# dcherednik/atracdenc

Hardware: AMD Instinct MI355X
Metric: ATRAC3 1024-sample stereo frames/sec (higher is better)
Workload: dtype f32; 1 GPU; ATRAC3 LP2 132 kbps stereo, 64 streams x 64 frames = 4096 frames per GPU per step (BASELINE configs[1]), 'noise' PCM resident in HBM, frames written to HBM (PCIe excluded); streams_per_gpu=64, frame_bytes=384, input=noise, tonal_components=True, parallelism=streams/1, launch=1 process x 1 GPU(s), one host thread and one at3hip context per device, collectives=none (no RCCL); start/stop barrier only

## Files before the change

### atracdenc_amd/csrc/at3_k_gain.hpp

```cpp
#pragma once
#include "at3_common.hpp"

namespace at3 {

struct GainParams {
    const float* sub;
    GainRec* rec;
    cpx* bins;
    BandState* state;
    Curve* curves;
    int n_blocks;
    int f0;
    int js;
    int n_streams;
    int literal;
};

constexpr int kLowCutBin = 38;

__device__ inline void median3_32(const float* in, float* out)
{
    for (int i = 0; i < 32; ++i) {
        const int lo = i > 0 ? i - 1 : 0;
        const int hi = i < 31 ? i + 1 : 31;
        if (hi - lo == 1) {
            out[i] = fmaxf(in[lo], in[hi]);
        } else {
            const float a = in[lo], b = in[lo + 1], c = in[hi];
            out[i] = fmaxf(fminf(a, b), fminf(fmaxf(a, b), c));
        }
    }
}

__device__ inline float curve_target(const float* in, const float* filtered)
{
    float maxRaw = 0.0f;
    for (int i = 0; i < 32; ++i) maxRaw = fmaxf(maxRaw, in[i]);
    float bestLevel = 0.0f;
    int bestEnd = -1;
    for (int j = 0; j + 3 <= 32; ++j) {
        const float minVal = fminf(fminf(filtered[j], filtered[j + 1]), filtered[j + 2]);
        if (minVal > bestLevel) {
            bestLevel = minVal;
            bestEnd = j + 2;
        }
    }
    float plateau = 0.0f;
    bool release = false;
    if (!(bestLevel < 1e-6f)) {
        plateau = bestLevel;
        while (bestEnd + 1 < 32 && filtered[bestEnd + 1] >= bestLevel) ++bestEnd;
        if (bestEnd < 31) {
            if (in[31] < bestLevel * 0.1f) {
                release = true;
            } else {
                bool anyHigh = false;
                for (int i = bestEnd + 1; i < 32; ++i)
                    if (in[i] >= bestLevel * 0.7f) {
                        anyHigh = true;
                        break;
                    }
                release = !anyHigh && (in[31] < bestLevel * 0.5f);
            }
        }
    }
    const bool usePlateau = plateau > 1e-6f && !release && plateau >= maxRaw * 0.4f;
    return usePlateau ? plateau : in[31];
}

__device__ __forceinline__ int irfft_pad(int i) { return i + (i >> 5); }

template <bool Z1>
__device__ __forceinline__ void bfly4_inv_sparse(f2& x0, f2& x1, f2& x2, f2& x3, f2 w1, f2 w3)
{
    const f2 s2 = pk_cmul(x3, w3);
    const f2 f0 = x0;
    if (Z1) {
        x2 = f0 - s2;
        x0 = f0 + s2;
        x1 = pk_sub_ib(f0, s2);
        x3 = pk_add_ib(f0, s2);
    } else {
        const f2 s0 = pk_cmul(x1, w1);
        const f2 s3 = s0 + s2, s4 = s0 - s2;
        x2 = f0 - s3;
        x0 = f0 + s3;
        x1 = pk_add_ib(f0, s4);
        x3 = pk_sub_ib(f0, s4);
    }
}

template <int KAPPA>
__device__ __forceinline__ void irfft_pass_2_8(cpx* F, const cpx* tw, int lane)
{
    cpx* B = F + 33 * lane + KAPPA;
    f2 x[16];
    const int r0 = (lane >> 4) + 4 * ((lane >> 2) & 3) + 16 * (lane & 3);
#pragma unroll
    for (int i = 0; i < 16; ++i) {
        const int r = r0 + 64 * (i >> 2);
        const bool nz = (i & 3) == 0 ? r >= 38 : (i & 3) == 1 ? r == 0 : (i & 3) == 3 ? r <= 218 : false;
        x[i] = f2{0.0f, 0.0f};
        if ((i & 3) != 2 && nz) x[i] = ld2(B + 2 * i);
    }
    const f2 a1 = ld2(tw + 256 * KAPPA), a3 = ld2(tw + 768 * KAPPA);
    bfly4_inv_sparse<false>(x[0], x[1], x[2], x[3], a1, a3);
#pragma unroll
    for (int g = 1; g < 4; ++g) bfly4_inv_sparse<true>(x[4 * g], x[4 * g + 1], x[4 * g + 2], x[4 * g + 3], a1, a3);
#pragma unroll
    for (int j = 0; j < 4; ++j) {
        const int k = KAPPA + 2 * j;
        bfly4<true>(x[j], x[j + 4], x[j + 8], x[j + 12], ld2(tw + 64 * k), ld2(tw + 128 * k), ld2(tw + 192 * k));
    }
#pragma unroll
    for (int i = 0; i < 16; ++i) st2(B + 2 * i, x[i]);
}

struct Tw32_128 {
    f2 a[3];
    f2 w[4][3];
};
__device__ __forceinline__ Tw32_128 irfft_tw_32_128(const cpx (*g)[128], int v)
{
    Tw32_128 t;
    t.a[0] = ld2(&g[0][v]);
    t.a[1] = ld2(&g[1][v]);
    t.a[2] = ld2(&g[2][v]);
#pragma unroll
    for (int j = 0; j < 4; ++j) {
        t.w[j][0] = ld2(&g[3 + 3 * j][v]);
        t.w[j][1] = ld2(&g[4 + 3 * j][v]);
        t.w[j][2] = ld2(&g[5 + 3 * j][v]);
    }
    return t;
}
__device__ __forceinline__ void irfft_pass_32_128(cpx* F, const Tw32_128& t, int v)
{
    const int k = v & 31, G2 = v >> 5;
    cpx* B = F + 528 * G2 + k;
    f2 x[16];
#pragma unroll
    for (int i = 0; i < 16; ++i) x[i] = ld2(B + 33 * i);
#pragma unroll
    for (int g = 0; g < 4; ++g) bfly4<true>(x[4 * g], x[4 * g + 1], x[4 * g + 2], x[4 * g + 3], t.a[0], t.a[1], t.a[2]);
#pragma unroll
    for (int j = 0; j < 4; ++j) bfly4<true>(x[j], x[j + 4], x[j + 8], x[j + 12], t.w[j][0], t.w[j][1], t.w[j][2]);
#pragma unroll
    for (int i = 0; i < 16; ++i) st2(B + 33 * i, x[i]);
}

template <int NT>
struct Tw512 {
    f2 w[512 / NT][3];
};
template <int NT>
__device__ __forceinline__ Tw512<NT> irfft_tw_512(const cpx (*g)[128], int tid)
{
    static_assert(NT == 128, "Tables::gain_tw is laid out for 128 work-items");
    Tw512<NT> t;
#pragma unroll
    for (int u = 0; u < 512 / NT; ++u) {
        t.w[u][0] = ld2(&g[15 + 3 * u][tid]);
        t.w[u][1] = ld2(&g[16 + 3 * u][tid]);
        t.w[u][2] = ld2(&g[17 + 3 * u][tid]);
    }
    return t;
}
template <int NT>
__device__ __forceinline__ void irfft_pass_512(cpx* F, const Tw512<NT>& t, int tid)
{
#pragma unroll
    for (int u0 = 0; u0 < 512 / NT; u0 += 4) {
        f2 x[4][4];
        cpx* B[4];
#pragma unroll
        for (int u = 0; u < 4; ++u) {
            B[u] = F + irfft_pad(tid + NT * (u0 + u));
#pragma unroll
            for (int q = 0; q < 4; ++q) x[u][q] = ld2(B[u] + 528 * q);
        }
#pragma unroll
        for (int u = 0; u < 4; ++u) bfly4<true>(x[u][0], x[u][1], x[u][2], x[u][3], t.w[u0 + u][0], t.w[u0 + u][1], t.w[u0 + u][2]);
#pragma unroll
        for (int u = 0; u < 4; ++u) {
            st2(B[u] + 528, x[u][1]);
            st2(B[u] + 1056, x[u][2]);
        }
    }
}

template <int CTRL>
__device__ __forceinline__ double dpp_f64_zero_fill(double v)
{
    const uint64_t b = (uint64_t)__double_as_longlong(v);
    const uint32_t lo = (uint32_t)AT3_DPP((uint32_t)b, CTRL, true), hi = (uint32_t)AT3_DPP((uint32_t)(b >> 32), CTRL, true);
    return __longlong_as_double((long long)(((uint64_t)hi << 32) | lo));
}
__device__ __forceinline__ double row_scan_add_f64(double v)
{
    v += dpp_f64_zero_fill<0x111>(v);
    v += dpp_f64_zero_fill<0x112>(v);
    v += dpp_f64_zero_fill<0x114>(v);
    v += dpp_f64_zero_fill<0x118>(v);
    return v;
}
constexpr int kGainBins = 220;

constexpr int kSpecRowStride = 18;
constexpr int kSpecItemBytes = 2432;
struct SpecItemLds {
    union {
        cpx x[16 * kSpecRowStride];
        double e[304];
    };
};
static_assert(sizeof(SpecItemLds) == kSpecItemBytes, "SpecItemLds layout");

__global__ __launch_bounds__(64) void k_gain_spec(GainParams p, const Tables* T, int n_items)
{
    __shared__ __attribute__((aligned(16))) SpecItemLds s_item[4];
    const int lane = threadIdx.x, row = lane >> 4, L = lane & 15;
    SpecItemLds& S = s_item[row];
    const int nfr = p.n_blocks - p.f0;
    const int quads = (nfr + 3) >> 2;
    int wg = blockIdx.x;
    const int band = wg % 3; wg /= 3;
    const int ch = wg % 2; wg /= 2;
    const int fr = 4 * (wg % quads) + row;
    const int s = wg / quads;
    const bool valid = fr < nfr;
    const int f = p.f0 + (valid ? fr : nfr - 1);
    const int item = (((s * nfr) + (f - p.f0)) * 2 + ch) * 3 + band;
    (void)n_items;
    const int cb = f - 1;
    const size_t sublen = (size_t)(p.n_blocks + 2) * 256;
    const float* sb0 = p.sub + ((size_t)s * 8 + 0 * 4 + band) * sublen + (size_t)(cb + 2) * 256 - 128;
    const float* sb1 = p.sub + ((size_t)s * 8 + 1 * 4 + band) * sublen + (size_t)(cb + 2) * 256 - 128;
    GainRec* rec = p.rec + (((size_t)s * p.n_blocks + f) * 2 + ch) * 3 + band;
    cpx* bins = p.bins + (size_t)item * kGainBins;

    f2 a[16];
    {
        f2 raw[16], rb[16], win[16];
#pragma unroll
        for (int t = 0; t < 16; ++t) {
            const int i = L + 16 * t;
            raw[t] = *reinterpret_cast<const f2*>((p.js || ch == 0 ? sb0 : sb1) + 2 * i);
            if (p.js) rb[t] = *reinterpret_cast<const f2*>(sb1 + 2 * i);
        }
#pragma unroll
        for (int t = 0; t < 16; ++t) win[t] = ld2(&T->spec16_win[t][L]);
        __builtin_amdgcn_sched_barrier(0);
#pragma unroll
        for (int t = 0; t < 16; ++t) {
            f2 v = raw[t];
            if (p.js) v = (ch == 0) ? (v + rb[t]) * mk2(0.5f, 0.5f) : (v - rb[t]) * mk2(0.5f, 0.5f);
            a[4 * (t & 3) + (t >> 2)] = v * win[t];
        }
    }
    f2 tw_l[15];
#pragma unroll
    for (int q = 0; q < 15; ++q) tw_l[q] = ld2(&T->spec16_tw[q][L]);
    __builtin_amdgcn_sched_barrier(0);
    {
        const f2 w0 = ld2(&T->tw256[0]);
#pragma unroll
        for (int q3 = 0; q3 < 4; ++q3) bfly4<false>(a[4 * q3], a[4 * q3 + 1], a[4 * q3 + 2], a[4 * q3 + 3], w0, w0, w0);
#pragma unroll
        for (int k = 0; k < 4; ++k)
            bfly4<false>(a[k], a[k + 4], a[k + 8], a[k + 12], ld2(&T->tw256[16 * k]), ld2(&T->tw256[32 * k]), ld2(&T->tw256[48 * k]));
    }
    f2 b[16];
    {
#pragma unroll
        for (int r = 0; r < 16; ++r) st2(&S.x[r * kSpecRowStride + L], a[r]);
        wave_sync();
        const float4* src = reinterpret_cast<const float4*>(&S.x[L * kSpecRowStride]);
#pragma unroll
        for (int m = 0; m < 8; ++m) {
            const float4 v = src[m];
            b[2 * m] = mk2(v.x, v.y);
            b[2 * m + 1] = mk2(v.z, v.w);
        }
        wave_sync();
    }
    {
        const f2 u1 = tw_l[0], u2 = tw_l[1], u3 = tw_l[2];
#pragma unroll
        for (int q1 = 0; q1 < 4; ++q1) bfly4<false>(b[q1], b[q1 + 4], b[q1 + 8], b[q1 + 12], u1, u2, u3);
#pragma unroll
        for (int j = 0; j < 4; ++j) bfly4<false>(b[4 * j], b[4 * j + 1], b[4 * j + 2], b[4 * j + 3], tw_l[3 + 3 * j], tw_l[4 + 3 * j], tw_l[5 + 3 * j]);
    }
    f2 fa[8], fb[8];
    f2 f128 = mk2(0.0f, 0.0f);
    {
        const int partner = 4 * ((lane & 48) | ((16 - L) & 15));
#pragma unroll
        for (int jj = 0; jj < 8; ++jj) {
            const int je = 15 - jj;
            const f2 pe = b[(je >> 2) + 4 * (je & 3)];
            f2 other;
            other.x = __uint_as_float((uint32_t)__builtin_amdgcn_ds_bpermute(partner, (int)__float_as_uint(pe.x)));
            other.y = __uint_as_float((uint32_t)__builtin_amdgcn_ds_bpermute(partner, (int)__float_as_uint(pe.y)));
            if (jj > 0) {
                const int j0 = 16 - jj;
                const f2 own = b[(j0 >> 2) + 4 * (j0 & 3)];
                if (L == 0) other = own;
            }
            const f2 fpk = b[(jj >> 2) + 4 * (jj & 3)];
            const cpx stw = T->spec16_stw[jj][L];
            const float fnr = other.x, fni = -other.y;
            const float f1r = fpk.x + fnr, f1i = fpk.y + fni;
            const float f2r = fpk.x - fnr, f2i = fpk.y - fni;
            const float twr = f2r * stw.r - f2i * stw.i, twi = f2r * stw.i + f2i * stw.r;
            fa[jj] = mk2((f1r + twr) * 0.5f, (f1i + twi) * 0.5f);
            fb[jj] = mk2((f1r - twr) * 0.5f, (twi - f1i) * 0.5f);
        }
        if (L == 0) {
            const f2 f0 = b[0];
            fa[0] = mk2(f0.x + f0.y, 0.0f);
            fb[0] = mk2(f0.x - f0.y, 0.0f);
        }
        {
            const f2 fpk = b[2];
            const cpx stw = T->spec16_stw[8][L];
            const float fnr = fpk.x, fni = -fpk.y;
            const float f1r = fpk.x + fnr, f1i = fpk.y + fni;
            const float f2r = fpk.x - fnr, f2i = fpk.y - fni;
            const float twr = f2r * stw.r - f2i * stw.i, twi = f2r * stw.i + f2i * stw.r;
            f128 = mk2((f1r - twr) * 0.5f, (twi - f1i) * 0.5f);
        }
    }
    if (valid) {
#pragma unroll
        for (int jj = 0; jj < 8; ++jj) {
            const int k = L + 16 * jj;
            if (k >= kLowCutBin) st2(&bins[k - kLowCutBin], fa[jj]);
            st2(&bins[256 - k - kLowCutBin], fb[jj]);
        }
        if (L == 0) st2(&bins[128 - kLowCutBin], f128);
    }
    bool fast_done = false;
    {
        const double h1 = (double)T->hpf_w[1], h2 = (double)T->hpf_w[2];
        double et = 0.0, ef = 0.0;
#pragma unroll
        for (int jj = 0; jj < 8; ++jj) {
            const int k = L + 16 * jj;
            const double ea = (double)fa[jj].x * fa[jj].x + (double)fa[jj].y * fa[jj].y;
            const double eb = (double)fb[jj].x * fb[jj].x + (double)fb[jj].y * fb[jj].y;
            et += ea;
            et += eb;
            const double wa = (k < kLowCutBin) ? 0.0 : (k == kLowCutBin) ? ea * h1 * h1 : (k == kLowCutBin + 1) ? ea * h2 * h2 : ea;
            ef += wa;
            ef += eb;
        }
        if (L == 0) {
            const double e128 = (double)f128.x * f128.x + (double)f128.y * f128.y;
            et += e128;
            ef += e128;
        }
        et = row_scan_add_f64(et);
        ef = row_scan_add_f64(ef);
        bool need = false;
        float hfr = 0.0f;
        if (L == 15) {
            if (et > 0.0 && ef > 0.0) {
                const double r = ef / et;
                hfr = (float)r;
                if (!(hfr >= 1e-30f)) {
                    need = true;
                } else {
                    const uint32_t hb = __float_as_uint(hfr);
                    const double below = ((double)__uint_as_float(hb - 1u) + (double)hfr) * 0.5, above = ((double)hfr + (double)__uint_as_float(hb + 1u)) * 0.5;
                    const double margin = r * 4e-13;
                    need = !(r - below > margin && above - r > margin);
                }
            }
        }
        if (p.literal || __ballot(need && valid) != 0ull) {
            fast_done = false;
        } else {
            if (valid && L == 15) rec->hfr = hfr;
            fast_done = true;
        }
    }
    if (fast_done) return;
    {
#pragma unroll
        for (int jj = 0; jj < 8; ++jj) {
            const int k = L + 16 * jj;
            S.e[k] = (double)fa[jj].x * fa[jj].x + (double)fa[jj].y * fa[jj].y;
            S.e[256 - k] = (double)fb[jj].x * fb[jj].x + (double)fb[jj].y * fb[jj].y;
        }
        if (L == 0) S.e[128] = (double)f128.x * f128.x + (double)f128.y * f128.y;
        for (int k = 257 + L; k < 304; k += 16) S.e[k] = 0.0;
    }
    wave_sync();
    double acc = 0.0;
    if (lane < 8) {
        const int it = lane >> 1, kind = lane & 1;
        const double* E = s_item[it].e;
        const double h1 = (double)T->hpf_w[1], h2 = (double)T->hpf_w[2];
        if (kind == 1) {
            acc += E[kLowCutBin] * h1 * h1;
            acc += E[kLowCutBin + 1] * h2 * h2;
        }
        const double* src = E + (kind ? kLowCutBin + 2 : 0);
        for (int k0 = 0; k0 < 256; k0 += 16) {
            double v[16];
#pragma unroll
            for (int i = 0; i < 16; ++i) v[i] = src[k0 + i];
#pragma unroll
            for (int i = 0; i < 16; ++i) acc += v[i];
        }
        acc += src[256];
    }
    const uint64_t ab = (uint64_t)__double_as_longlong(acc);
    const int alo = (int)(uint32_t)ab, ahi = (int)(uint32_t)(ab >> 32);
    const uint64_t fb64 = (uint64_t)(uint32_t)__builtin_amdgcn_ds_bpermute(4 * (2 * row + 1), alo) |
                          ((uint64_t)(uint32_t)__builtin_amdgcn_ds_bpermute(4 * (2 * row + 1), ahi) << 32);
    const uint64_t tb64 = (uint64_t)(uint32_t)__builtin_amdgcn_ds_bpermute(4 * (2 * row), alo) |
                          ((uint64_t)(uint32_t)__builtin_amdgcn_ds_bpermute(4 * (2 * row), ahi) << 32);
    if (valid && L == 0) {
        const double totalE = __longlong_as_double((long long)tb64), filtE = __longlong_as_double((long long)fb64);
        rec->hfr = (totalE > 0.0) ? (float)(filtE / totalE) : 0.0f;
    }
}

struct GainLds {
    cpx f[2048 + 64];
};

__global__ __launch_bounds__(128) void k_gain_analysis(GainParams p, const Tables* __restrict__ T)
{
    __shared__ __attribute__((aligned(16))) GainLds s_item[1];
    const int tid = threadIdx.x, wave = __builtin_amdgcn_readfirstlane((int)(threadIdx.x >> 6)), lane = threadIdx.x & 63;
    GainLds& L = s_item[0];
    const int nfr = p.n_blocks - p.f0;
    const bool valid = true;
    int wg = blockIdx.x;
    const size_t item = blockIdx.x;
    const int band = wg % 3; wg /= 3;
    const int ch = wg % 2; wg /= 2;
    const int f = p.f0 + wg % nfr;
    const int s = wg / nfr;
    GainRec* rec = p.rec + (((size_t)s * p.n_blocks + f) * 2 + ch) * 3 + band;
    const float hfr = rec->hfr;
    const cpx* bins = p.bins + item * kGainBins;
    const int k0 = kLowCutBin + tid, k1 = kLowCutBin + 128 + tid;
    const cpx bin0 = bins[tid];
    const cpx bin1 = bins[k1 <= 256 ? 128 + tid : tid];
    const cpx stw_in0 = T->stw2048[k0 - 1];
    const cpx stw_in1 = T->stw2048[k1 - 1 < 1024 ? k1 - 1 : 1023];
    const float hpf1 = T->hpf_w[1], hpf2 = T->hpf_w[2];
    __builtin_amdgcn_sched_barrier(0);
    if (hfr < 0.05f) return;
    __builtin_amdgcn_sched_barrier(0);
    const Tw32_128 tw_b = irfft_tw_32_128(T->gain_tw, tid);
    const Tw512<128> tw_c = irfft_tw_512<128>(T->gain_tw, tid);
    __builtin_amdgcn_sched_barrier(0);
#pragma unroll
    for (int q = 0; q < 2; ++q) {
        const int k = q ? k1 : k0;
        const cpx fr = q ? bin1 : bin0;
        cpx fk;
        const float scale = 8.0f;
        if (k == 256) {
            fk.r = fr.r * scale * 0.5f;
            fk.i = 0.0f;
        } else if (k >= kLowCutBin + 2) {
            fk.r = fr.r * scale;
            fk.i = fr.i * scale;
        } else {
            const float w = (k == kLowCutBin) ? hpf1 : hpf2;
            fk.r = fr.r * scale * w;
            fk.i = fr.i * scale * w;
        }
        const cpx fok = cmul(fk, q ? stw_in1 : stw_in0);
        cpx a, b, nb;
        a.r = fk.r + fok.r; a.i = fk.i + fok.i;
        b.r = fk.r - fok.r; b.i = -(fk.i - fok.i);
        nb.r = 0.0f - b.r; nb.i = 0.0f - b.i;
        if (k <= 256) {
            const int pa = fft_leaf_pos<2048>(k);
            L.f[irfft_pad(pa)] = a;
            L.f[irfft_pad(pa) + 1] = a;
            const int pb = fft_leaf_pos<2048>(2048 - k);
            L.f[irfft_pad(pb) - 1] = b;
            L.f[irfft_pad(pb)] = nb;
        }
    }
    __syncthreads();

    if (wave == 0) irfft_pass_2_8<0>(L.f, T->tw2048, lane);
    else irfft_pass_2_8<1>(L.f, T->tw2048, lane);
    __syncthreads();

    irfft_pass_32_128(L.f, tw_b, tid);
    __syncthreads();

    irfft_pass_512<128>(L.f, tw_c, tid);
    __syncthreads();


    const float norm = 1.0f / 4096.0f;
    float* s_micro = reinterpret_cast<float*>(L.f);
#pragma unroll
    for (int q = 0; q < 2; ++q) {
        const int n = tid + 128 * q;
        const int c = (n & 3) | ((n & 0xc) << 1) | ((n & 0x10) >> 2) | (n & 0xe0);
        cpx* src = L.f + 528 + 4 * c + (c >> 3);
        float acc = 0.0f;
#pragma unroll
        for (int i = 0; i < 4; ++i) {
            const f2 v = ld2(src + i) * norm;
            const f2 sq = v * v;
            st2(src + i, sq);
            acc += sq.x;
            acc += sq.y;
        }
        acc /= 8;
        s_micro[c] = sqrtf(acc);
    }
    __syncthreads();
    if (tid < 32) {
        const cpx* src = L.f + 528 + 33 * lane;
        f2 x[32];
#pragma unroll
        for (int i = 0; i < 32; ++i) x[i] = ld2(src + i);
        float acc = 0.0f;
#pragma unroll
        for (int i = 0; i < 32; ++i) {
            acc += x[i].x;
            acc += x[i].y;
        }
        acc /= 64;
        rec->gain[lane] = sqrtf(acc);
    } else if (wave == 1 && lane < 32) {
        const float4 ma = *reinterpret_cast<const float4*>(s_micro + 8 * lane), mb = *reinterpret_cast<const float4*>(s_micro + 8 * lane + 4);
        float m[8] = {ma.x, ma.y, ma.z, ma.w, mb.x, mb.y, mb.z, mb.w};
#pragma unroll
        for (int i = 1; i < 8; ++i) {
#pragma unroll
            for (int k = i; k > 0; --k) {
                const float lo = fminf(m[k - 1], m[k]), hi = fmaxf(m[k - 1], m[k]);
                m[k - 1] = lo;
                m[k] = hi;
            }
        }
        rec->lo[lane] = m[2];
        rec->hi[lane] = m[6];
    }
}

constexpr int kGa1RowStride = 18;
constexpr int kGa1RowSlots = 16 * kGa1RowStride + 16;
constexpr int kGa1SubStride = 33;
struct Gain1Lds {
    union {
        cpx x[4 * kGa1RowSlots];
        struct {
            cpx out[32 * kGa1SubStride];
            float micro[256];
        };
    };
};
static_assert(sizeof(Gain1Lds) <= 10240, "sixteen items per CU");

struct PermPair {
    int a, b;
};
__device__ __forceinline__ PermPair perm32_swap(int a, int b)
{
    const auto r = __builtin_amdgcn_permlane32_swap(a, b, false, false);
    return PermPair{(int)r[0], (int)r[1]};
}
__device__ __forceinline__ PermPair perm16_swap(int a, int b)
{
    const auto r = __builtin_amdgcn_permlane16_swap(a, b, false, false);
    return PermPair{(int)r[0], (int)r[1]};
}
template <bool WIDE>
__device__ __forceinline__ void swap_f2(f2& a, f2& b)
{
    const PermPair x = WIDE ? perm32_swap((int)__float_as_uint(a.x), (int)__float_as_uint(b.x)) : perm16_swap((int)__float_as_uint(a.x), (int)__float_as_uint(b.x));
    const PermPair y = WIDE ? perm32_swap((int)__float_as_uint(a.y), (int)__float_as_uint(b.y)) : perm16_swap((int)__float_as_uint(a.y), (int)__float_as_uint(b.y));
    a = mk2(__uint_as_float((uint32_t)x.a), __uint_as_float((uint32_t)y.a));
    b = mk2(__uint_as_float((uint32_t)x.b), __uint_as_float((uint32_t)y.b));
}

__global__ __launch_bounds__(64) AT3_WAVES_PER_EU(4) void k_gain_analysis1(GainParams p, const Tables* T)
{
    __shared__ __attribute__((aligned(16))) Gain1Lds L;
    const int lane = threadIdx.x, R = lane >> 4, j = lane & 15;
    const int nfr = p.n_blocks - p.f0;
    int wg = blockIdx.x;
    const size_t item = blockIdx.x;
    const int band = wg % 3; wg /= 3;
    const int ch = wg % 2; wg /= 2;
    const int f = p.f0 + wg % nfr;
    const int s = wg / nfr;
    GainRec* rec = p.rec + (((size_t)s * p.n_blocks + f) * 2 + ch) * 3 + band;
    const float hfr = rec->hfr;
    if (hfr < 0.05f) return;
    const cpx* bins = p.bins + item * kGainBins;
    const cpx* tw = T->tw2048;

#define AT3_STAGE() __builtin_amdgcn_sched_barrier(0)
    const int r0 = (lane >> 4) + 4 * ((lane >> 2) & 3) + 16 * (lane & 3);
    cpx ba[4], bb[4], sa[4], sb[4], b256 = {0.0f, 0.0f}, s256 = {0.0f, 0.0f};
#pragma unroll
    for (int q = 0; q < 4; ++q) {
        const int ka = r0 + 64 * q, kb = 256 - r0 - 64 * q;
        const int kac = ka >= kLowCutBin ? ka : kLowCutBin, kbc = kb >= kLowCutBin ? kb : kLowCutBin;
        ba[q] = bins[kac - kLowCutBin];
        sa[q] = T->stw2048[kac - 1];
        bb[q] = bins[kbc - kLowCutBin];
        sb[q] = T->stw2048[kbc - 1];
    }
    if (lane == 0) {
        b256 = bins[256 - kLowCutBin];
        s256 = T->stw2048[255];
    }
    const float hpf1 = T->hpf_w[1], hpf2 = T->hpf_w[2];
    f2 a1[2], a3[2], w8[2][4][3];
#pragma unroll
    for (int kappa = 0; kappa < 2; ++kappa) {
        a1[kappa] = ld2(tw + 256 * kappa);
        a3[kappa] = ld2(tw + 768 * kappa);
#pragma unroll
        for (int jj = 0; jj < 4; ++jj) {
            const int k = kappa + 2 * jj;
            w8[kappa][jj][0] = ld2(tw + 64 * k);
            w8[kappa][jj][1] = ld2(tw + 128 * k);
            w8[kappa][jj][2] = ld2(tw + 192 * k);
        }
    }
    f2 twb[15];
#pragma unroll
    for (int sl = 0; sl < 15; ++sl) twb[sl] = ld2(&T->ga1_twb[0][sl][j]);
    AT3_STAGE();
    f2 la[4], lb[4], la256 = mk2(0.0f, 0.0f);
    {
        auto leaf = [&](cpx fr, cpx stw, int k, bool want_b) -> f2 {
            cpx fk;
            const float scale = 8.0f;
            if (k == 256) {
                fk.r = fr.r * scale * 0.5f;
                fk.i = 0.0f;
            } else if (k >= kLowCutBin + 2) {
                fk.r = fr.r * scale;
                fk.i = fr.i * scale;
            } else {
                const float w = (k == kLowCutBin) ? hpf1 : hpf2;
                fk.r = fr.r * scale * w;
                fk.i = fr.i * scale * w;
            }
            const cpx fok = cmul(fk, stw);
            return want_b ? mk2(fk.r - fok.r, -(fk.i - fok.i)) : mk2(fk.r + fok.r, fk.i + fok.i);
        };
#pragma unroll
        for (int q = 0; q < 4; ++q) {
            const int ka = r0 + 64 * q, kb = 256 - r0 - 64 * q;
            la[q] = (ka >= kLowCutBin) ? leaf(ba[q], sa[q], ka, false) : mk2(0.0f, 0.0f);
            lb[q] = (kb >= kLowCutBin) ? leaf(bb[q], sb[q], kb, true) : mk2(0.0f, 0.0f);
        }
        if (lane == 0) la256 = leaf(b256, s256, 256, false);
    }
    f2 y[2][16];
    f2 twc[2][4][3];
#pragma unroll
    for (int kappa = 0; kappa < 2; ++kappa) {
        f2 x[16];
#pragma unroll
        for (int i = 0; i < 16; ++i) x[i] = mk2(0.0f, 0.0f);
#pragma unroll
        for (int q = 0; q < 4; ++q) {
            x[4 * q] = la[q];
            x[4 * q + 3] = kappa ? mk2(0.0f - lb[q].x, 0.0f - lb[q].y) : lb[q];
        }
        x[1] = la256;
        bfly4_inv_sparse<false>(x[0], x[1], x[2], x[3], a1[kappa], a3[kappa]);
#pragma unroll
        for (int g = 1; g < 4; ++g) bfly4_inv_sparse<true>(x[4 * g], x[4 * g + 1], x[4 * g + 2], x[4 * g + 3], a1[kappa], a3[kappa]);
#pragma unroll
        for (int jj = 0; jj < 4; ++jj) bfly4<true>(x[jj], x[jj + 4], x[jj + 8], x[jj + 12], w8[kappa][jj][0], w8[kappa][jj][1], w8[kappa][jj][2]);
        cpx* row = L.x + R * kGa1RowSlots;
#pragma unroll
        for (int i = 0; i < 16; ++i) st2(row + i * kGa1RowStride + j, x[i]);
        wave_sync();
        f2 b[16];
        {
            const float4* src = reinterpret_cast<const float4*>(row + j * kGa1RowStride);
#pragma unroll
            for (int m = 0; m < 8; ++m) {
                const float4 v = src[m];
                b[2 * m] = mk2(v.x, v.y);
                b[2 * m + 1] = mk2(v.z, v.w);
            }
        }
        wave_sync();
#pragma unroll
        for (int g = 0; g < 4; ++g) bfly4<true>(b[4 * g], b[4 * g + 1], b[4 * g + 2], b[4 * g + 3], twb[0], twb[1], twb[2]);
#pragma unroll
        for (int jj = 0; jj < 4; ++jj) bfly4<true>(b[jj], b[jj + 4], b[jj + 8], b[jj + 12], twb[3 + 3 * jj], twb[4 + 3 * jj], twb[5 + 3 * jj]);
#pragma unroll
        for (int i = 0; i < 16; ++i) y[kappa][i] = b[i];
        AT3_STAGE();
        if (kappa == 0) {
#pragma unroll
            for (int sl = 0; sl < 15; ++sl) twb[sl] = ld2(&T->ga1_twb[1][sl][j]);
        } else {
#pragma unroll
            for (int u = 0; u < 2; ++u)
#pragma unroll
                for (int t = 0; t < 4; ++t)
#pragma unroll
                    for (int q = 0; q < 3; ++q) twc[u][t][q] = ld2(&T->ga1_twc[4 * u + t][q][lane]);
        }
        AT3_STAGE();
    }
#pragma unroll
    for (int u = 0; u < 2; ++u)
#pragma unroll
        for (int t = 0; t < 8; ++t) swap_f2<true>(y[u][t], y[u][8 + t]);
#pragma unroll
    for (int u = 0; u < 2; ++u)
#pragma unroll
        for (int t = 0; t < 4; ++t) {
            swap_f2<false>(y[u][t], y[u][4 + t]);
            swap_f2<false>(y[u][8 + t], y[u][12 + t]);
        }
#pragma unroll
    for (int u = 0; u < 2; ++u)
#pragma unroll
        for (int t = 0; t < 4; ++t) {
            const int i = 4 * R + t;
            bfly4<true>(y[u][t], y[u][4 + t], y[u][8 + t], y[u][12 + t], twc[u][t][0], twc[u][t][1], twc[u][t][2]);
            st2(L.out + kGa1SubStride * i + 2 * j + u, y[u][4 + t]);
            st2(L.out + kGa1SubStride * (16 + i) + 2 * j + u, y[u][8 + t]);
        }
    wave_sync();
    const float norm = 1.0f / 4096.0f;
#pragma unroll
    for (int q = 0; q < 4; ++q) {
        const int n = lane + 64 * q;
        const int c = (n & 3) | ((n & 0xc) << 1) | ((n & 0x10) >> 2) | (n & 0xe0);
        const cpx* src = L.out + 4 * c + (c >> 3);
        float acc = 0.0f;
#pragma unroll
        for (int i = 0; i < 4; ++i) {
            const f2 v = ld2(src + i) * norm;
            const f2 sq = v * v;
            acc += sq.x;
            acc += sq.y;
        }
        acc /= 8;
        L.micro[c] = sqrtf(acc);
    }
    wave_sync();
    if (lane < 32) {
        const cpx* src = L.out + kGa1SubStride * lane;
        f2 x[32];
#pragma unroll
        for (int i = 0; i < 32; ++i) x[i] = ld2(src + i);
        float acc = 0.0f;
#pragma unroll
        for (int i = 0; i < 32; ++i) {
            const f2 v = x[i] * norm;
            const f2 sq = v * v;
            acc += sq.x;
            acc += sq.y;
        }
        acc /= 64;
        rec->gain[lane] = sqrtf(acc);
    } else {
        const int sf = lane - 32;
        const float4 ma = *reinterpret_cast<const float4*>(L.micro + 8 * sf), mb = *reinterpret_cast<const float4*>(L.micro + 8 * sf + 4);
        float m[8] = {ma.x, ma.y, ma.z, ma.w, mb.x, mb.y, mb.z, mb.w};
#pragma unroll
        for (int i = 1; i < 8; ++i) {
#pragma unroll
            for (int k = i; k > 0; --k) {
                const float lo = fminf(m[k - 1], m[k]), hi = fmaxf(m[k - 1], m[k]);
                m[k - 1] = lo;
                m[k] = hi;
            }
        }
        rec->lo[sf] = m[2];
        rec->hi[sf] = m[6];
    }
}

__global__ __launch_bounds__(256) void k_gain_tail(GainParams p, int n_items)
{
    __shared__ float s_g[8][32], s_f[8][32], s_m[8][32];
    const int tid = threadIdx.x, grp = tid >> 5, j = tid & 31, half = grp & 1;
    const int nfr = p.n_blocks - p.f0;
    int item = blockIdx.x * 8 + grp;
    const bool valid = item < n_items;
    if (!valid) item = n_items - 1;
    int wg = item;
    const int band = wg % 3; wg /= 3;
    const int ch = wg % 2; wg /= 2;
    const int f = p.f0 + wg % nfr;
    const int s = wg / nfr;
    GainRec* rec = p.rec + (((size_t)s * p.n_blocks + f) * 2 + ch) * 3 + band;
    const float hfr = rec->hfr;
    const float g_j = rec->gain[j];
    asm volatile("" ::"v"(g_j));
    const bool active = valid && !(hfr < 0.05f);
    if (__ballot(active) == 0ull) return;
    float* s_gain = s_g[grp];
    float* s_filt = s_f[grp];
    float* s_minv = s_m[grp];
    const float in_j = active ? g_j : 0.0f;
    s_gain[j] = in_j;
    wave_sync();
    float filt_j;
    {
        const float a = s_gain[j > 0 ? j - 1 : 0], c = s_gain[j < 31 ? j + 1 : 31];
        if (j == 0) filt_j = fmaxf(in_j, c);
        else if (j == 31) filt_j = fmaxf(a, in_j);
        else filt_j = fmaxf(fminf(a, in_j), fminf(fmaxf(a, in_j), c));
    }
    s_filt[j] = filt_j;
    wave_sync();
    s_minv[j] = (j <= 29) ? fminf(fminf(filt_j, s_filt[j < 30 ? j + 1 : 31]), s_filt[j < 30 ? j + 2 : 31]) : -1.0f;
    wave_sync();
    float maxRaw = 0.0f, sum = 0.0f, bestLevel = 0.0f;
    int bestEnd = -1;
    for (int k = 0; k < 32; ++k) {
        const float g = s_gain[k];
        maxRaw = fmaxf(maxRaw, g);
        sum += g;
        const float mv = s_minv[k];
        if (k <= 29 && mv > bestLevel) {
            bestLevel = mv;
            bestEnd = k + 2;
        }
    }
    const uint32_t ge = (uint32_t)(__ballot(filt_j >= bestLevel) >> (32 * half));
    const uint32_t high = (uint32_t)(__ballot(in_j >= bestLevel * 0.7f) >> (32 * half));
    const float last = s_gain[31];
    float plateau = 0.0f;
    bool release = false;
    if (!(bestLevel < 1e-6f)) {
        plateau = bestLevel;
        const uint32_t x = (bestEnd + 1 < 32) ? (ge >> (bestEnd + 1)) : 0u;
        bestEnd += (x == 0xffffffffu) ? 32 : __builtin_ctz(~x);
        if (bestEnd < 31) {
            if (last < bestLevel * 0.1f) release = true;
            else release = ((high >> (bestEnd + 1)) == 0u) && (last < bestLevel * 0.5f);
        }
    }
    const bool usePlateau = plateau > 1e-6f && !release && plateau >= maxRaw * 0.4f;
    if (active && j == 0) {
        rec->cur_hpf = sum / 32.0f;
        rec->target = usePlateau ? plateau : last;
    }
}

constexpr int kScanChunk = 512;
__global__ __launch_bounds__(64) void k_gain_scan(GainParams p, int n_streams)
{
    __shared__ float s_hfr[kScanChunk], s_g31[kScanChunk], s_tgt[kScanChunk], s_hpf[kScanChunk];
    const int lane = threadIdx.x;
    const int idx = blockIdx.x;
    if (idx >= n_streams * 6) return;
    const int band = idx % 3, ch = (idx / 3) % 2, s = idx / 6;
    BandState* st = p.state + (size_t)s * 8 + ch * 4 + band;
    float lvl = st->last_level, tgt = st->last_target, hpf = st->last_hpf;
    const int nfr = p.n_blocks - p.f0;
    for (int base = 0; base < nfr; base += kScanChunk) {
        const int cnt = (nfr - base < kScanChunk) ? nfr - base : kScanChunk;
        for (int i = lane; i < cnt; i += 64) {
            const GainRec* rec = p.rec + (((size_t)s * p.n_blocks + p.f0 + base + i) * 2 + ch) * 3 + band;
            s_hfr[i] = rec->hfr;
            s_g31[i] = rec->gain[31];
            s_tgt[i] = rec->target;
            s_hpf[i] = rec->cur_hpf;
        }
        __syncthreads();
        if (lane == 0) {
            for (int i = 0; i < cnt; ++i) {
                const float h = s_hfr[i], g = s_g31[i], t = s_tgt[i], e = s_hpf[i];
                s_g31[i] = lvl;
                s_tgt[i] = tgt;
                s_hpf[i] = hpf;
                if (h < 0.05f) {
                    lvl = 0.0f;
                } else {
// ... 456 lines not shown
```

### atracdenc_amd/csrc/at3_tables.cpp

```cpp
#include "at3_tables.hpp"
#include "at1_tables.hpp"
#include "at3p_tables.hpp"

#include <cmath>
#include <cstring>

#define AT3_RUNTIME_LIBM __attribute__((optnone, noinline))

namespace at3 {

extern const float kTapHalf[24];
const float kTapHalf[24] = {
    -0.00001461907,  -0.00009205479, -0.000056157569, 0.00030117269, 0.0002422519,  -0.00085293897,
    -0.0005205574,   0.0020340169,   0.00078333891,   -0.0042153862, -0.00075614988, 0.0078402944,
    -0.000061169922, -0.01344162,    0.0024626821,    0.021736089,   -0.007801671,   -0.034090221,
    0.01880949,      0.054326009,    -0.043596379,    -0.099384367,  0.13207909,     0.46424159};

namespace {

#include "at3_libm64.inc"

const short kAthMilliBel[] = {
    9669, 9669, 9626, 9512, 9353, 9113, 8882, 8676, 8469, 8243, 7997, 7748, 7492, 7239, 7000, 6762, 6529, 6302, 6084, 5900,
    5717, 5534, 5351, 5167, 5004, 4812, 4638, 4466, 4310, 4173, 4050, 3922, 3723, 3577, 3451, 3281, 3132, 3036, 2902, 2760,
    2658, 2591, 2441, 2301, 2212, 2125, 2018, 1900, 1770, 1682, 1594, 1512, 1430, 1341, 1260, 1198, 1136, 1057, 998,  943,
    887,  846,  744,  712,  693,  668,  637,  606,  580,  555,  529,  502,  475,  448,  422,  398,  375,  351,  327,  322,
    312,  301,  291,  268,  246,  215,  182,  146,  107,  61,   13,   -35,  -96,  -156, -179, -235, -295, -350, -401, -421,
    -446, -499, -532, -535, -513, -476, -431, -313, -179, 8,    203,  403,  580,  736,  881,  1022, 1154, 1251, 1348, 1421,
    1479, 1399, 1285, 1193, 1287, 1519, 1914, 2369, 3352, 4352, 5352, 6352, 7352, 8352, 9352, 9999, 9999, 9999, 9999, 9999};

const uint16_t kBfuStart[33] = {0,   8,   16,  24,  32,  40,  48,  56,  64,  80,  96,  112, 128, 144, 160, 176, 192,
                                224, 256, 288, 320, 352, 384, 416, 448, 480, 512, 576, 640, 704, 768, 896, 1024};

}

AT3_RUNTIME_LIBM float ath_db(float freq)
{
    if (freq < 10.) freq = 10.;
    if (freq > 29853.) freq = 29853.;
    const double fl = 40. * log10(0.1 * freq);
    const unsigned idx = (unsigned)fl;
    return 0.01 * (kAthMilliBel[idx] * (1 + idx - fl) + kAthMilliBel[idx + 1] * (fl - idx));
}

AT3_RUNTIME_LIBM void fill_twiddles(cpx* tw, int n, bool inverse)
{
    const double pi = 3.141592653589793238462643383279502884197169399375105820974944;
    for (int i = 0; i < n; ++i) {
        double phase = -2 * pi * i / n;
        if (inverse) phase *= -1;
        tw[i].r = (float)cos(phase);
        tw[i].i = (float)sin(phase);
    }
}

AT3_RUNTIME_LIBM void mdct_sincos(float* dst, size_t n, float scale)
{
    const float alpha = 2.0 * M_PI / (8.0 * n);
    const float omiga = 2.0 * M_PI / n;
    scale = sqrtf(scale / n);
    for (size_t i = 0; i < (n >> 2); ++i) {
        dst[2 * i + 0] = scale * cosf(omiga * i + alpha);
        dst[2 * i + 1] = scale * sinf(omiga * i + alpha);
    }
}

namespace {

AT3_RUNTIME_LIBM void fill_super_twiddles(cpx* tw, int ncfft, bool inverse)
{
    for (int i = 0; i < ncfft / 2; ++i) {
        double phase = -3.14159265358979323846264338327 * ((double)(i + 1) / ncfft + .5);
        if (inverse) phase *= -1;
        tw[i].r = (float)cos(phase);
        tw[i].i = (float)sin(phase);
    }
}

}

AT3_RUNTIME_LIBM void build_tables(Tables* t)
{
    memset(t, 0, sizeof(*t));
    for (int i = 0; i < 24; ++i) t->qmf_win[i] = t->qmf_win[47 - i] = kTapHalf[i] * 2.0;
    for (uint32_t i = 0; i < 64; ++i) t->scale[i] = pow(2.0, (double)(i / 3.0 - 21.0));
    for (int i = 0; i < 256; ++i) t->enc_win[i] = (sin(((i + 0.5) / 256.0 - 0.5) * M_PI) + 1.0);
    for (int i = 0; i < 16; ++i) t->gain_level[i] = pow(2.0, 4 - i);
    for (int i = 0; i < 31; ++i) t->gain_interp[i] = pow(2.0, -1.0 / 8 * (i - 15));

    mdct_sincos(t->mdct_sincos, 512, 1.0f);
    fill_twiddles(t->tw128, 128, false);
    fill_twiddles(t->tw256, 256, false);
    fill_twiddles(t->tw2048, 2048, true);
    fill_super_twiddles(t->stw256, 256, false);
    fill_super_twiddles(t->stw2048, 2048, true);
    for (int L = 0; L < 16; ++L) {
        for (int q = 1; q <= 3; ++q) t->spec16_tw[q - 1][L] = t->tw256[4 * q * L];
        for (int j = 0; j < 4; ++j)
            for (int q = 1; q <= 3; ++q) t->spec16_tw[3 + 3 * j + q - 1][L] = t->tw256[q * (L + 16 * j)];
        for (int jj = 0; jj < 9; ++jj) {
            const int k = L + 16 * jj;
            cpx z = {0.0f, 0.0f};
            if (k >= 1 && k <= 128 && (jj < 8 || L == 0)) z = t->stw256[k - 1];
            t->spec16_stw[jj][L] = z;
        }
    }
    for (int tid = 0; tid < 128; ++tid) {
        const int k = tid & 31;
        for (int q = 0; q < 3; ++q) t->gain_tw[q][tid] = t->tw2048[16 * (q + 1) * k];
        for (int j = 0; j < 4; ++j)
            for (int q = 0; q < 3; ++q) t->gain_tw[3 + 3 * j + q][tid] = t->tw2048[4 * (q + 1) * (k + 32 * j)];
        for (int u = 0; u < 4; ++u)
            for (int q = 0; q < 3; ++q) t->gain_tw[15 + 3 * u + q][tid] = t->tw2048[(q + 1) * (tid + 128 * u)];
    }

    for (int u = 0; u < 2; ++u)
        for (int j = 0; j < 16; ++j) {
            const int k = 2 * j + u;
            for (int q = 0; q < 3; ++q) t->ga1_twb[u][q][j] = t->tw2048[16 * (q + 1) * k];
            for (int jj = 0; jj < 4; ++jj)
                for (int q = 0; q < 3; ++q) t->ga1_twb[u][3 + 3 * jj + q][j] = t->tw2048[4 * (q + 1) * (k + 32 * jj)];
        }
    for (int lane = 0; lane < 64; ++lane)
        for (int u = 0; u < 2; ++u)
            for (int tt = 0; tt < 4; ++tt) {
                const int kk = 2 * (lane & 15) + u + 32 * (4 * (lane >> 4) + tt);
                for (int q = 0; q < 3; ++q) t->ga1_twc[4 * u + tt][q][lane] = t->tw2048[(q + 1) * kk];
            }

    for (int en = 0; en < 18; ++en)
        for (int L = 0; L < 16; ++L) {
            const int q1 = L >> 2, q2 = L & 3, b = q1 + 4 * q2;
            float* v = t->mdct_tab[en][L];
            if (en < 4) {
                const int e = 2 * b + 32 * en;
                v[0] = t->enc_win[e]; v[1] = t->enc_win[128 + e]; v[2] = t->enc_win[127 - e]; v[3] = t->enc_win[255 - e];
            } else if (en < 8) {
                const int n = 2 * (b + 16 * (en - 4));
                v[0] = t->mdct_sincos[n]; v[1] = t->mdct_sincos[n + 1]; v[2] = t->mdct_sincos[n + 128]; v[3] = t->mdct_sincos[n + 129];
            } else if (en < 12) {
                const int n = 2 * (8 * q1 + 2 * q2 + 32 * (en - 8));
                v[0] = t->mdct_sincos[n]; v[1] = t->mdct_sincos[n + 1]; v[2] = t->mdct_sincos[n + 2]; v[3] = t->mdct_sincos[n + 3];
            } else if (en < 15) {
                const int j = en - 11, k = 2 * q2;
                v[0] = t->tw128[4 * j * k].r; v[1] = t->tw128[4 * j * k].i; v[2] = t->tw128[4 * j * (k + 1)].r; v[3] = t->tw128[4 * j * (k + 1)].i;
            } else {
                const int j = en - 14, k = 8 * q1 + 2 * q2;
                v[0] = t->tw128[j * k].r; v[1] = t->tw128[j * k].i; v[2] = t->tw128[j * (k + 1)].r; v[3] = t->tw128[j * (k + 1)].i;
            }
        }

    {
        const float eN = 0.15f * 512.0f;
        const float fN = 512.0f;
        for (int n = 0; n < 512; ++n) {
            const float fn = (float)n;
            if (n == 0) {
                t->planck[n] = 0.0f;
            } else if (fn < eN) {
                const float z = eN * (1.0f / fn + 1.0f / (fn - eN));
                t->planck[n] = 1.0f / (1.0f + expf(z));
            } else if (fn <= fN - eN) {
                t->planck[n] = 1.0f;
            } else {
                const float m = fN - fn;
                const float z = eN * (1.0f / m + 1.0f / (m - eN));
                t->planck[n] = 1.0f / (1.0f + expf(z));
            }
        }
        for (int i = 0; i < 3; ++i) t->hpf_w[i] = 0.5f * (1.0f - cosf((float)M_PI * i / 2.0f));
    }
    for (int L = 0; L < 16; ++L)
        for (int tt = 0; tt < 16; ++tt) {
            const int i = L + 16 * tt;
            t->spec16_win[tt][L].r = t->planck[2 * i];
            t->spec16_win[tt][L].i = t->planck[2 * i + 1];
        }

    for (size_t i = 0; i < 1024; ++i) {
        float f = (float)(i + 3) * 0.5 * 44100 / (float)1024;
        float v = log10f(f) - 3.5;
        v = -10 * v * v + 3 - f / 3000;
        v = pow(10, (0.1 * v));
        t->loud_curve[i] = v;
    }
    {
        float ath_line[1024];
        const float mf = (float)44100 / 2000.0;
        for (size_t i = 0; i < 1024; ++i) {
            const float f = (float)(i + 1) * mf / 1024;
            float trh = ath_db(1.e3 * f) - 100;
            trh -= f * f * 0.015;
            ath_line[i] = trh;
        }
        for (int b = 0; b < 32; ++b) {
            float x = 999;
            for (int line = kBfuStart[b]; line < kBfuStart[b + 1]; ++line) x = fminf(x, ath_line[line]);
            x = pow(10, 0.1f * x);
            t->ath_bfu[b] = x;
        }
    }
    static const double tab[16][2] = {
        {0x1.661ec79f8f3bep+0, -0x1.efec65b963019p-2}, {0x1.571ed4aaf883dp+0, -0x1.b0b6832d4fca4p-2},
        {0x1.49539f0f010b0p+0, -0x1.7418b0a1fb77bp-2}, {0x1.3c995b0b80385p+0, -0x1.39de91a6dcf7bp-2},
        {0x1.30d190c8864a5p+0, -0x1.01d9bf3f2b631p-2}, {0x1.25e227b0b8ea0p+0, -0x1.97c1d1b3b7af0p-3},
        {0x1.1bb4a4a1a343fp+0, -0x1.2f9e393af3c9fp-3}, {0x1.12358f08ae5bap+0, -0x1.960cbbf788d5cp-4},
        {0x1.0953f419900a7p+0, -0x1.a6f9db6475fcep-5}, {0x1.0000000000000p+0, 0x0.0p+0},
        {0x1.e608cfd9a47acp-1, 0x1.338ca9f24f53dp-4},  {0x1.ca4b31f026aa0p-1, 0x1.476a9543891bap-3},
        {0x1.b2036576afce6p-1, 0x1.e840b4ac4e4d2p-3},  {0x1.9c2d163a1aa2dp-1, 0x1.40645f0c6651cp-2},
        {0x1.886e6037841edp-1, 0x1.88e9c2c1b9ff8p-2},  {0x1.767dcf5534862p-1, 0x1.ce0a44eb17bccp-2}};
    static const double poly[4] = {-0x1.712b6f70a7e4dp-2, 0x1.ecabf496832e0p-2, -0x1.715479ffae3dep-1,
                                   0x1.715475f35c8b8p+0};
    memcpy(t->log2f_tab, tab, sizeof(tab));
    memcpy(t->log2f_poly, poly, sizeof(poly));
    memcpy(t->libm.log_c, kLogData, sizeof(t->libm.log_c));
    memcpy(t->libm.log_tab, kLogData + 18, sizeof(t->libm.log_tab));
    memcpy(t->libm.exp_c, kExpData, sizeof(t->libm.exp_c));
    memcpy(t->libm.exp_tab, kExpTab, sizeof(t->libm.exp_tab));
}

}

namespace at1 {

namespace {

const uint16_t kSpecsStartLong[kMaxBfus] = {0,   8,   16,  24,  32,  36,  40,  44,  48,  56,  64,  72,  80,  86,  92,  98,  104, 110,
                                            116, 122, 128, 134, 140, 146, 152, 159, 166, 173, 180, 189, 198, 207, 216, 226, 236, 246,
                                            256, 268, 280, 292, 304, 316, 328, 340, 352, 372, 392, 412, 432, 452, 472, 492};
const uint8_t kSpecsPerBlock[kMaxBfus] = {8,  8,  8,  8,  4,  4,  4,  4,  8,  8,  8,  8,  6,  6,  6,  6,  6,  6,
                                          6,  6,  6,  6,  6,  6,  7,  7,  7,  7,  9,  9,  9,  9,  10, 10, 10, 10,
                                          12, 12, 12, 12, 12, 12, 12, 12, 20, 20, 20, 20, 20, 20, 20, 20};

}

AT3_RUNTIME_LIBM void build_tables(Tables* t)
{
    memset(t, 0, sizeof(*t));
    for (int i = 0; i < 24; ++i) t->qmf_win[i] = t->qmf_win[47 - i] = at3::kTapHalf[i] * 2.0;
    for (uint32_t i = 0; i < 64; ++i) t->scale[i] = pow(2.0, (double)(i / 3.0 - 21.0));
    for (uint32_t i = 0; i < 32; ++i) t->sine[i] = sin((i + 0.5) * (M_PI / (2.0 * 32.0)));
    at3::mdct_sincos(t->sc512, 512, 1.0f);
    at3::mdct_sincos(t->sc256, 256, 0.5f);
    at3::mdct_sincos(t->sc64, 64, 0.5f);
    at3::fill_twiddles(t->tw128, 128, false);
    at3::fill_twiddles(t->tw64, 64, false);
    at3::fill_twiddles(t->tw16, 16, false);
    for (size_t i = 0; i < 512; ++i) {
        float f = (float)(i + 3) * 0.5 * 44100 / (float)512;
        float v = log10f(f) - 3.5;
        v = -10 * v * v + 3 - f / 3000;
        v = pow(10, (0.1 * v));
        t->loud[i] = v;
    }
    {
        float ath_line[512];
        const float mf = (float)44100 / 2000.0;
        for (size_t i = 0; i < 512; ++i) {
            const float f = (float)(i + 1) * mf / 512;
            float trh = at3::ath_db(1.e3 * f) - 100;
            trh -= f * f * 0.015;
            ath_line[i] = trh;
        }
        for (int b = 0; b < kMaxBfus; ++b) {
            float x = 999;
            for (int line = kSpecsStartLong[b]; line < kSpecsStartLong[b] + kSpecsPerBlock[b]; ++line) x = fmin(x, ath_line[line]);
            x = pow(10, 0.1 * x);
            t->ath_bfu[b] = x;
        }
    }
    static const float fir[10] = {-8.65163e-18 * 2.0, -0.00851586 * 2.0, -6.74764e-18 * 2.0, 0.0209036 * 2.0, -3.36639e-17 * 2.0,
                                  -0.0438162 * 2.0,   -1.54175e-17 * 2.0, 0.0931738 * 2.0,   -5.52212e-17 * 2.0, -0.313819 * 2.0};
    memcpy(t->fir, fir, sizeof(fir));
    static const float fix_long[kMaxBfus] = {7, 7, 7, 6, 6, 6, 6, 6, 6, 6, 6, 6, 6, 6, 6, 6, 6, 6, 6, 6, 6, 6, 5, 5, 5, 5,
                                             5, 5, 5, 5, 5, 5, 5, 5, 5, 4, 4, 4, 3, 3, 3, 3, 3, 3, 2, 1, 1, 1, 1, 0, 0, 0};
    static const float fix_short[kMaxBfus] = {6, 6, 6, 6, 6, 6, 6, 6, 6, 6, 6, 6, 6, 6, 6, 6, 6, 6, 6, 6, 6, 6, 6, 6, 5, 5,
                                              5, 5, 5, 5, 5, 5, 5, 5, 5, 5, 4, 4, 4, 4, 4, 4, 4, 4, 0, 0, 0, 0, 0, 0, 0, 0};
    memcpy(t->fix_long, fix_long, sizeof(fix_long));
    memcpy(t->fix_short, fix_short, sizeof(fix_short));
    static const double tab[16][2] = {
        {0x1.661ec79f8f3bep+0, -0x1.57bf7808caadep-2}, {0x1.571ed4aaf883dp+0, -0x1.2bef0a7c06ddbp-2},
        {0x1.49539f0f010b0p+0, -0x1.01eae7f513a67p-2}, {0x1.3c995b0b80385p+0, -0x1.b31d8a68224e9p-3},
        {0x1.30d190c8864a5p+0, -0x1.6574f0ac07758p-3}, {0x1.25e227b0b8ea0p+0, -0x1.1aa2bc79c8100p-3},
        {0x1.1bb4a4a1a343fp+0, -0x1.a4e76ce8c0e5ep-4}, {0x1.12358f08ae5bap+0, -0x1.1973c5a611cccp-4},
        {0x1.0953f419900a7p+0, -0x1.252f438e10c1ep-5}, {0x1.0000000000000p+0, 0x0.0p+0},
        {0x1.e608cfd9a47acp-1, 0x1.aa5aa5df25984p-5},  {0x1.ca4b31f026aa0p-1, 0x1.c5e53aa362eb4p-4},
        {0x1.b2036576afce6p-1, 0x1.526e57720db08p-3},  {0x1.9c2d163a1aa2dp-1, 0x1.bc2860d224770p-3},
        {0x1.886e6037841edp-1, 0x1.1058bc8a07ee1p-2},  {0x1.767dcf5534862p-1, 0x1.4043057b6ee09p-2}};
    memcpy(t->logf_tab, tab, sizeof(tab));
    t->logf_ln2 = 0x1.62e42fefa39efp-1;
    t->logf_poly[0] = -0x1.00ea348b88334p-2;
    t->logf_poly[1] = 0x1.5575b0be00b6ap-2;
    t->logf_poly[2] = -0x1.ffffef20a4123p-2;
}

}

namespace at3p {

namespace {

const float kFir[384] = {
#include "at3p_fir.inc"
};

}

AT3_RUNTIME_LIBM void build_tables(Tables* t)
{
    memset(t, 0, sizeof(*t));
    memcpy(t->fir, kFir, sizeof(kFir));
    const float dct_scale = 32.0 * (float)(128 * 512.0);
    at3::mdct_sincos(t->sc32, 32, dct_scale / 2);
    at3::mdct_sincos(t->sc256, 256, 1.0f);
    at3::fill_twiddles(t->tw8, 8, false);
    at3::fill_twiddles(t->tw64, 64, false);
    for (size_t i = 0; i < 128; i++) t->sine128[i] = 2.0 * sinf((i + 0.5) * (M_PI / (2.0 * 128)));
    for (size_t i = 0; i < 64; i++) t->sine64[i] = 2.0 * sinf((i + 0.5) * (M_PI / (2.0 * 64)));
}

}
```

Baseline: 15.69 million frames/s.

## Fuse last two iRFFT passes in gain kernel using permlane swaps

Merges the radix-16 32x128 pass and the final radix-4 512 pass of the gain-analysis inverse FFT into one register-resident pass. Data is exchanged between lanes with permlane32/permlane16 swaps instead of going through LDS, which removes one barrier and one LDS round trip. The squaring and normalisation are folded into the fused pass's stores, so the energy loop only reads. The twiddle table layout is remapped to the new thread-to-data assignment, and correctness depends on that mapping being exact.

```diff
diff --git a/atracdenc_amd/csrc/at3_k_gain.hpp b/atracdenc_amd/csrc/at3_k_gain.hpp
--- a/atracdenc_amd/csrc/at3_k_gain.hpp
+++ b/atracdenc_amd/csrc/at3_k_gain.hpp
@@ -116,76 +116,84 @@
     for (int i = 0; i < 16; ++i) st2(B + 2 * i, x[i]);
 }
 
+struct PermPair {
+    int a, b;
+};
+__device__ __forceinline__ PermPair perm32_swap(int a, int b)
+{
+    const auto r = __builtin_amdgcn_permlane32_swap(a, b, false, false);
+    return PermPair{(int)r[0], (int)r[1]};
+}
+__device__ __forceinline__ PermPair perm16_swap(int a, int b)
+{
+    const auto r = __builtin_amdgcn_permlane16_swap(a, b, false, false);
+    return PermPair{(int)r[0], (int)r[1]};
+}
+template <bool WIDE>
+__device__ __forceinline__ void swap_f2(f2& a, f2& b)
+{
+    const PermPair x = WIDE ? perm32_swap((int)__float_as_uint(a.x), (int)__float_as_uint(b.x)) : perm16_swap((int)__float_as_uint(a.x), (int)__float_as_uint(b.x));
+    const PermPair y = WIDE ? perm32_swap((int)__float_as_uint(a.y), (int)__float_as_uint(b.y)) : perm16_swap((int)__float_as_uint(a.y), (int)__float_as_uint(b.y));
+    a = mk2(__uint_as_float((uint32_t)x.a), __uint_as_float((uint32_t)y.a));
+    b = mk2(__uint_as_float((uint32_t)x.b), __uint_as_float((uint32_t)y.b));
+}
+
 struct Tw32_128 {
     f2 a[3];
     f2 w[4][3];
 };
-__device__ __forceinline__ Tw32_128 irfft_tw_32_128(const cpx (*g)[128], int v)
+__device__ __forceinline__ Tw32_128 irfft_tw_32_128(const cpx (*g)[128], int tid)
 {
     Tw32_128 t;
-    t.a[0] = ld2(&g[0][v]);
-    t.a[1] = ld2(&g[1][v]);
-    t.a[2] = ld2(&g[2][v]);
+    t.a[0] = ld2(&g[0][tid]);
+    t.a[1] = ld2(&g[1][tid]);
+    t.a[2] = ld2(&g[2][tid]);
 #pragma unroll
     for (int j = 0; j < 4; ++j) {
-        t.w[j][0] = ld2(&g[3 + 3 * j][v]);
-        t.w[j][1] = ld2(&g[4 + 3 * j][v]);
-        t.w[j][2] = ld2(&g[5 + 3 * j][v]);
+        t.w[j][0] = ld2(&g[3 + 3 * j][tid]);
+        t.w[j][1] = ld2(&g[4 + 3 * j][tid]);
+        t.w[j][2] = ld2(&g[5 + 3 * j][tid]);
     }
     return t;
 }
-__device__ __forceinline__ void irfft_pass_32_128(cpx* F, const Tw32_128& t, int v)
-{
-    const int k = v & 31, G2 = v >> 5;
-    cpx* B = F + 528 * G2 + k;
-    f2 x[16];
-#pragma unroll
-    for (int i = 0; i < 16; ++i) x[i] = ld2(B + 33 * i);
-#pragma unroll
-    for (int g = 0; g < 4; ++g) bfly4<true>(x[4 * g], x[4 * g + 1], x[4 * g + 2], x[4 * g + 3], t.a[0], t.a[1], t.a[2]);
-#pragma unroll
-    for (int j = 0; j < 4; ++j) bfly4<true>(x[j], x[j + 4], x[j + 8], x[j + 12], t.w[j][0], t.w[j][1], t.w[j][2]);
-#pragma unroll
-    for (int i = 0; i < 16; ++i) st2(B + 33 * i, x[i]);
-}
-
-template <int NT>
 struct Tw512 {
-    f2 w[512 / NT][3];
+    f2 w[4][3];
 };
-template <int NT>
-__device__ __forceinline__ Tw512<NT> irfft_tw_512(const cpx (*g)[128], int tid)
-{
-    static_assert(NT == 128, "Tables::gain_tw is laid out for 128 work-items");
-    Tw512<NT> t;
-#pragma unroll
-    for (int u = 0; u < 512 / NT; ++u) {
+__device__ __forceinline__ Tw512 irfft_tw_512(const cpx (*g)[128], int tid)
+{
+    Tw512 t;
+#pragma unroll
+    for (int u = 0; u < 4; ++u) {
         t.w[u][0] = ld2(&g[15 + 3 * u][tid]);
         t.w[u][1] = ld2(&g[16 + 3 * u][tid]);
         t.w[u][2] = ld2(&g[17 + 3 * u][tid]);
     }
     return t;
 }
-template <int NT>
-__device__ __forceinline__ void irfft_pass_512(cpx* F, const Tw512<NT>& t, int tid)
-{
-#pragma unroll
-    for (int u0 = 0; u0 < 512 / NT; u0 += 4) {
-        f2 x[4][4];
-        cpx* B[4];
-#pragma unroll
-        for (int u = 0; u < 4; ++u) {
-            B[u] = F + irfft_pad(tid + NT * (u0 + u));
-#pragma unroll
-            for (int q = 0; q < 4; ++q) x[u][q] = ld2(B[u] + 528 * q);
-        }
-#pragma unroll
-        for (int u = 0; u < 4; ++u) bfly4<true>(x[u][0], x[u][1], x[u][2], x[u][3], t.w[u0 + u][0], t.w[u0 + u][1], t.w[u0 + u][2]);
-#pragma unroll
-        for (int u = 0; u < 4; ++u) {
-            st2(B[u] + 528, x[u][1]);
-            st2(B[u] + 1056, x[u][2]);
-        }
+__device__ __forceinline__ void irfft_pass_32_128_512(cpx* F, const Tw32_128& tb, const Tw512& tc, int k, int R, float norm)
+{
+    const cpx* B = F + 528 * R + k;
+    f2 x[16];
+#pragma unroll
+    for (int i = 0; i < 16; ++i) x[i] = ld2(B + 33 * i);
+#pragma unroll
+    for (int g = 0; g < 4; ++g) bfly4<true>(x[4 * g], x[4 * g + 1], x[4 * g + 2], x[4 * g + 3], tb.a[0], tb.a[1], tb.a[2]);
+#pragma unroll
+    for (int j = 0; j < 4; ++j) bfly4<true>(x[j], x[j + 4], x[j + 8], x[j + 12], tb.w[j][0], tb.w[j][1], tb.w[j][2]);
+#pragma unroll
+    for (int t = 0; t < 8; ++t) swap_f2<true>(x[t], x[8 + t]);
+#pragma unroll
+    for (int t = 0; t < 4; ++t) {
+        swap_f2<false>(x[t], x[4 + t]);
+        swap_f2<false>(x[8 + t], x[12 + t]);
+    }
+    cpx* O = F + 528 + 132 * R + k;
+#pragma unroll
+    for (int t = 0; t < 4; ++t) {
+        bfly4<true>(x[t], x[4 + t], x[8 + t], x[12 + t], tc.w[t][0], tc.w[t][1], tc.w[t][2]);
+        const f2 v1 = x[4 + t] * norm, v2 = x[8 + t] * norm;
+        st2(O + 33 * t, v1 * v1);
+        st2(O + 33 * t + 528, v2 * v2);
     }
 }
 
@@ -458,7 +466,7 @@
     if (hfr < 0.05f) return;
     __builtin_amdgcn_sched_barrier(0);
     const Tw32_128 tw_b = irfft_tw_32_128(T->gain_tw, tid);
-    const Tw512<128> tw_c = irfft_tw_512<128>(T->gain_tw, tid);
+    const Tw512 tw_c = irfft_tw_512(T->gain_tw, tid);
     __builtin_amdgcn_sched_barrier(0);
 #pragma unroll
     for (int q = 0; q < 2; ++q) {
@@ -492,33 +500,27 @@
         }
     }
     __syncthreads();
-
     if (wave == 0) irfft_pass_2_8<0>(L.f, T->tw2048, lane);
     else irfft_pass_2_8<1>(L.f, T->tw2048, lane);
     __syncthreads();
 
-    irfft_pass_32_128(L.f, tw_b, tid);
+    irfft_pass_32_128_512(L.f, tw_b, tw_c, 16 * wave + (lane & 15), lane >> 4, 1.0f / 4096.0f);
     __syncthreads();
 
-    irfft_pass_512<128>(L.f, tw_c, tid);
-    __syncthreads();
-
-
-    const float norm = 1.0f / 4096.0f;
     float* s_micro = reinterpret_cast<float*>(L.f);
 #pragma unroll
     for (int q = 0; q < 2; ++q) {
         const int n = tid + 128 * q;
         const int c = (n & 3) | ((n & 0xc) << 1) | ((n & 0x10) >> 2) | (n & 0xe0);
-        cpx* src = L.f + 528 + 4 * c + (c >> 3);
+        const cpx* src = L.f + 528 + 4 * c + (c >> 3);
+        f2 sq[4];
+#pragma unroll
+        for (int i = 0; i < 4; ++i) sq[i] = ld2(src + i);
         float acc = 0.0f;
 #pragma unroll
         for (int i = 0; i < 4; ++i) {
-            const f2 v = ld2(src + i) * norm;
-            const f2 sq = v * v;
-            st2(src + i, sq);
-            acc += sq.x;
-            acc += sq.y;
+            acc += sq[i].x;
+            acc += sq[i].y;
         }
         acc /= 8;
         s_micro[c] = sqrtf(acc);
@@ -567,28 +569,6 @@
     };
 };
 static_assert(sizeof(Gain1Lds) <= 10240, "sixteen items per CU");
-
-struct PermPair {
-    int a, b;
-};
-__device__ __forceinline__ PermPair perm32_swap(int a, int b)
-{
-    const auto r = __builtin_amdgcn_permlane32_swap(a, b, false, false);
-    return PermPair{(int)r[0], (int)r[1]};
-}
-__device__ __forceinline__ PermPair perm16_swap(int a, int b)
-{
-    const auto r = __builtin_amdgcn_permlane16_swap(a, b, false, false);
-    return PermPair{(int)r[0], (int)r[1]};
-}
-template <bool WIDE>
-__device__ __forceinline__ void swap_f2(f2& a, f2& b)
-{
-    const PermPair x = WIDE ? perm32_swap((int)__float_as_uint(a.x), (int)__float_as_uint(b.x)) : perm16_swap((int)__float_as_uint(a.x), (int)__float_as_uint(b.x));
-    const PermPair y = WIDE ? perm32_swap((int)__float_as_uint(a.y), (int)__float_as_uint(b.y)) : perm16_swap((int)__float_as_uint(a.y), (int)__float_as_uint(b.y));
-    a = mk2(__uint_as_float((uint32_t)x.a), __uint_as_float((uint32_t)y.a));
-    b = mk2(__uint_as_float((uint32_t)x.b), __uint_as_float((uint32_t)y.b));
-}
 
 __global__ __launch_bounds__(64) AT3_WAVES_PER_EU(4) void k_gain_analysis1(GainParams p, const Tables* T)
 {
diff --git a/atracdenc_amd/csrc/at3_tables.cpp b/atracdenc_amd/csrc/at3_tables.cpp
--- a/atracdenc_amd/csrc/at3_tables.cpp
+++ b/atracdenc_amd/csrc/at3_tables.cpp
@@ -106,12 +106,12 @@
         }
     }
     for (int tid = 0; tid < 128; ++tid) {
-        const int k = tid & 31;
+        const int k = 16 * (tid >> 6) + (tid & 15), R = (tid >> 4) & 3;
         for (int q = 0; q < 3; ++q) t->gain_tw[q][tid] = t->tw2048[16 * (q + 1) * k];
         for (int j = 0; j < 4; ++j)
             for (int q = 0; q < 3; ++q) t->gain_tw[3 + 3 * j + q][tid] = t->tw2048[4 * (q + 1) * (k + 32 * j)];
         for (int u = 0; u < 4; ++u)
-            for (int q = 0; q < 3; ++q) t->gain_tw[15 + 3 * u + q][tid] = t->tw2048[(q + 1) * (tid + 128 * u)];
+            for (int q = 0; q < 3; ++q) t->gain_tw[15 + 3 * u + q][tid] = t->tw2048[(q + 1) * (k + 32 * (4 * R + u))];
     }
 
     for (int u = 0; u < 2; ++u)
```

Result: faster. 15.89 million frames/s (median of 4 runs) (+1.3%).
